# jtdaugherty/flux

Hardware: AMD Instinct MI355X
Metric: Msamples/sec on demo2.yml (fixed spp) (higher is better)
Workload: dtype f64

## Files before the change

flux_amd/_lib.py:

```python
import ctypes as C
import os

_HERE = os.path.dirname(os.path.abspath(__file__))
LIB_PATH = os.environ.get("FLUX_HIP_LIB") or os.path.join(_HERE, "libflux_hip.so")

FLUX_OK = 0
E_INVALID, E_DEVICE, E_NOMEM, E_IO = -1, -2, -3, -4
SHAPE_SPHERE, SHAPE_PLANE, SHAPE_DISK, SHAPE_BOX = 0, 1, 2, 3
MAT_MATTE, MAT_EMISSIVE, MAT_REFLECTIVE, MAT_GLOSSY = 0, 1, 2, 3
MAT_DIELECTRIC = 4
KERNEL_DEFAULT, KERNEL_STATIC, KERNEL_REFILL, KERNEL_SPLIT = 0, 1, 2, 3
MATH_FAST, MATH_STRICT = 0, 1
SAMPLER_REGULAR, SAMPLER_JITTERED, SAMPLER_MULTI_JITTERED, SAMPLER_CORRELATED_MULTI_JITTERED = 0, 1, 2, 3
TABLE_PIXEL, TABLE_DISC, TABLE_HEMI = 0, 1, 2
TRAVERSE_BVH, TRAVERSE_BRUTE, TRAVERSE_BVH_BINARY = 0, 1, 2
NUM_STATS = 16
BVH_INFO_WORDS = 16
PLAN_WORDS = 8
PLAN_NONE, PLAN_STATIC, PLAN_REFILL, PLAN_SPLIT, PLAN_BVH_BINARY, PLAN_BVH4 = -1, 0, 1, 2, 3, 4
ROUTE_NONE, ROUTE_TO_STRICT, ROUTE_KEPT_FAST = 0, 1, 2
PLAN_FLAG_TYP, PLAN_FLAG_MAX32, PLAN_FLAG_HITQ, PLAN_FLAG_TPUT_TABLE = 0x1, 0x2, 0x4, 0x8
PLAN_FLAG_DEPTH_CUT, PLAN_FLAG_UNIFORM_A, PLAN_FLAG_LDS_SCENE, PLAN_FLAG_TRIS = 0x10, 0x20, 0x40, 0x80
PLAN_FLAG_AXIS_SHIFT, PLAN_FLAG_AXIS_MASK = 8, 0x300
PLAN_FLAG_HQ_BITS_SHIFT, PLAN_FLAG_HQ_BITS_MASK = 10, 0xfc00
PLAN_FLAG_COPY_SHIFT, PLAN_FLAG_COPY_MASK = 16, 0x30000
CREATE_TIMING_WORDS = 8
CREATE_TIMING_NAMES = ("total", "host", "runtime", "alloc", "upload", "tables", "free", "other")
SHARD_AUTO, SHARD_SETS, SHARD_ROWS = 0, 1, 2
SHARD_LOOPBACK = 0x100
MULTI_INFO_WORDS = 8
MULTI_TIMING_WORDS = 8
ABI_VERSION = 3
AOV_CHANNELS = 8
AOV_ALBEDO_OFFSET, AOV_NORMAL_OFFSET, AOV_DEPTH, AOV_COVERAGE = 0, 3, 6, 7
AOV_ALBEDO, AOV_NORMAL = slice(AOV_ALBEDO_OFFSET, AOV_ALBEDO_OFFSET + 3), slice(AOV_NORMAL_OFFSET, AOV_NORMAL_OFFSET + 3)
MOMENT_CHANNELS = 8
MOMENT_RGB_OFFSET, MOMENT_VAR, MOMENT_MEAN_OFFSET, MOMENT_S2 = 0, 3, 4, 7
# ... 164 lines not shown
```

flux_amd/build.py:

```python
import os
import shutil
import subprocess
import sys

ROOT = os.path.dirname(os.path.dirname(os.path.abspath(__file__)))
CSRC = os.path.join(ROOT, "flux_amd", "csrc")
HIP_SOURCES = ["abi.hip", "multi.hip", "tables.hip", "render.hip", "denoise.hip", "adaptive.hip", "bvh.cpp", "scene_build.cpp", "launch_plan.cpp"]
HIP_HEADERS = ["flux_ctx.h", "scene_build.h", "joining_thread.h", "flux_device.h", "flux_plan.h", "flux_rng.h", "flux_tables.h", "flux_bvh.h", "flux_math.h",
               "flux_math_coeffs.h", "flux_env_verdict.h", "flux_plane_axis.h", "flux_moments.h", "render_body.inc", "aov_body.inc", "moments_body.inc", "adaptive_body.inc", "aov_chain_body.inc"]
HIP_LIB = os.path.join(ROOT, "flux_amd", "libflux_hip.so")

HIP_FLAGS = ["--offload-arch=gfx950", "-O3", "-std=c++17", "-fPIC", "-shared", "-ffp-contract=off",
             "-fno-fast-math", "-Wall", "-Wno-unused-function",
             "-mllvm", "-disable-machine-licm"]


def _newer(target, deps):
    if not os.path.exists(target):
        return True
    t = os.path.getmtime(target)
    return any(os.path.getmtime(d) > t for d in deps)


def _hipcc():
    for cand in (os.environ.get("HIPCC"), shutil.which("hipcc"), "/opt/rocm/bin/hipcc"):
        if cand and os.path.exists(cand):
            return cand
    raise RuntimeError("hipcc not found (set HIPCC)")


KERNEL_FILES = ["render.hip", "render_body.inc", "aov_body.inc", "moments_body.inc", "adaptive_body.inc", "aov_chain_body.inc", "tables.hip", "denoise.hip", "adaptive.hip", "flux_device.h", "flux_plan.h", "flux_bvh.h", "flux_math.h",
                "flux_math_coeffs.h", "flux_rng.h", "flux_tables.h", "flux_env_verdict.h", "flux_plane_axis.h", "flux_moments.h"]


def build_id(extra_flags=()):
    import hashlib

    def digest(names):
        h = hashlib.sha256()
        h.update(" ".join(HIP_FLAGS + list(extra_flags)).encode())
        for n in names:
            path = os.path.join(ROOT, "include", n) if n == "flux_abi.h" else os.path.join(CSRC, n)
            h.update(n.encode() + b"\0")
            with open(path, "rb") as f:
                h.update(f.read())
        return h.hexdigest()[:16]
    return f"lib:{digest(sorted(set(HIP_SOURCES + HIP_HEADERS + ['flux_abi.h'])))} kernels:{digest(KERNEL_FILES)}"


def _id_flag(extra_flags=()):
    return "-DFLUX_BUILD_ID=\"" + build_id(extra_flags) + "\""


def build_variant(out_path, extra_flags, verbose=False):
    srcs = [os.path.join(CSRC, s) for s in HIP_SOURCES]
# ... 48 lines not shown
```

flux_amd/csrc/abi.hip:

```cpp
#include <hip/hip_runtime.h>

#include <chrono>
#include <cmath>
#include <cstdarg>
#include <cstdio>
#include <cstring>
#include <memory>
#include <new>
#include <algorithm>
#include <cstdlib>
#include <string>
#include <vector>

#include "../../include/flux_abi.h"
#include "flux_device.h"
#include "flux_tables.h"
#include "flux_math_coeffs.h"

#include "flux_ctx.h"

namespace flux {

thread_local std::string g_last_error;

// ... 184 lines not shown
    const char *tables_env = std::getenv("FLUX_SAMPLE_TABLES");
    const int gx_stride = (tables_env && std::atoi(tables_env) == 0) ? 0 : h.rp.gx_stride;
    if (gx_stride) {
        alloc(c->d_glossx, own * c->N * (size_t)gx_stride);
        alloc_copy(c->d_gxoff, h.gx_off);
    }
    int tput_bits = 0;
    bool tput_finite = false;
    {
        RenderParams job = h.rp;
        job.nsamp = c->N;
        job.max_depth = (int32_t)c->D;
        const char *tput_env = std::getenv("FLUX_THROUGHPUT_TABLE");
        if (tput_table_bytes(job, &tput_bits)) {
            std::vector<double> tput;
            build_tput_table(h, tput_bits, (int)c->D, tput);
            tput_finite = tput_products_finite(h, tput_bits, (int)c->D, tput);
            if (!(tput_env && std::atoi(tput_env) == 0)) alloc_copy(c->d_tput, tput);
        }
    }
    std::vector<unsigned char> lobe_entries;
    const size_t lobe_bytes = lobe_frame_table(h, lobe_entries);
    if (lobe_bytes) alloc(c->d_lobe, lobe_bytes);
    alloc(c->d_setrows, own * sizeof(DevSetRows));
    alloc(c->d_rowperm, perm_bytes);
    alloc(c->d_invperm, perm_bytes);
    alloc(c->d_stats, FLUX_NUM_STATS * sizeof(unsigned long long));
    if (!h.tris.empty()) {
        alloc_copy(c->d_tris, h.tris);
        alloc_copy(c->d_nodes, h.nodes);
        alloc_copy(c->d_nodesq, h.nodesq);
        if (!h.arena.empty()) alloc_copy(c->d_arena, h.arena);
    }
    if (e == hipSuccess) e = hipMemset(c->d_stats, 0, FLUX_NUM_STATS * sizeof(unsigned long long));
    laps.lap(FLUX_CREATE_MS_UPLOAD);
    if (e == hipSuccess) e = c->ev0.create();
    if (e == hipSuccess) e = c->ev1.create();
    laps.lap(FLUX_CREATE_MS_OTHER);
    double tab_ms[3] = {0, 0, 0};
    if (e == hipSuccess)
        e = generate_tables(seed, c->S, c->sets, c->D, c->n, c->H, c->d_pix, c->d_disc, c->d_hemi, c->d_rowperm, c->d_invperm, nullptr, tab_ms);
    if (e == hipSuccess) {
        e = generate_gloss_table(c->d_pix, (size_t)c->sets.count * c->N, c->d_gloss, nullptr);
        if (e == hipSuccess && gx_stride)
            e = generate_glossx_table(c->d_gloss, (size_t)c->sets.count * c->N, h.gx_inv_e1.data(), h.rp.n_gloss_exp, gx_stride / 16,
                                      c->d_glossx, nullptr);
        if (e == hipSuccess && c->d_lobe)
            e = generate_lobe_frame_table(reinterpret_cast<const DevHitRec *>(c->d_fscene + h.fs.rec), (int)lobe_entries.size(), c->d_lobe, nullptr);
        if (e == hipSuccess) e = hipStreamSynchronize(nullptr);
    }
    laps.lap(FLUX_CREATE_MS_TABLES);
    laps.ms[FLUX_CREATE_MS_TABLES] -= tab_ms[0] + tab_ms[2];
    laps.ms[FLUX_CREATE_MS_ALLOC] += tab_ms[0];
    laps.ms[FLUX_CREATE_MS_FREE] += tab_ms[2];
    if (e == hipSuccess) {
        std::vector<DevSetRows> rows(own, DevSetRows{});
        for (size_t m = 0; m < own; m++) {
            rows[m].pix = c->d_pix + m * c->N;
            rows[m].disc = c->d_disc + m * c->N;
            rows[m].hemi = c->d_hemi + m * c->D * c->N * kHemiDoubles;
            rows[m].gloss = c->d_gloss + m * c->N * 4;
            rows[m].glossx = gx_stride ? c->d_glossx + m * c->N * (size_t)(gx_stride / 16) : nullptr;
        }
        copy(c->d_setrows, rows);
    }
    if (e != hipSuccess)
        return fail(e == hipErrorOutOfMemory ? FLUX_E_NOMEM : FLUX_E_DEVICE, "flux_ctx_create: %s", hipGetErrorString(e));

    RenderParams &rp = c->rp;
    rp = h.rp;
    rp.pixel_denom = 1.0 / (double)((uint64_t)c->n * c->n);
    rp.max_depth = (int32_t)c->D;
    rp.nsamp = c->N;
    rp.shapes = c->d_shapes;
    rp.mats = c->d_mats;
    rp.pix = c->d_pix;
    rp.disc = c->d_disc;
    rp.hemi = c->d_hemi;
    rp.gloss = c->d_gloss;
    rp.glossx = c->d_glossx;
    rp.gx_off = c->d_gxoff;
    rp.gx_stride = gx_stride;
    rp.tput = c->d_tput;
    rp.tput_bits = c->d_tput ? tput_bits : 0;
// ... 587 lines not shown
    return FLUX_OK;
}

int flux_ctx_copy_table(flux_ctx *ctx, int which, double *out, uint64_t out_doubles) {
    if (!ctx || !out) return fail(FLUX_E_INVALID, "null argument");
    DeviceGuard guard(ctx->device);
    const size_t SN = (size_t)ctx->sets.count * ctx->N;
    if (which == FLUX_TABLE_PIXEL || which == FLUX_TABLE_DISC) {
        if (out_doubles < SN * 2) return fail(FLUX_E_INVALID, "output too small: need %zu doubles", SN * 2);
        HIP_TRY(hipMemcpy(out, which == FLUX_TABLE_PIXEL ? ctx->d_pix : ctx->d_disc, SN * 2 * sizeof(double),
                          hipMemcpyDeviceToHost));
        return FLUX_OK;
    }
    if (which == FLUX_TABLE_HEMI) {
        const size_t total = SN * ctx->D * 3;
        if (out_doubles < total) return fail(FLUX_E_INVALID, "output too small: need %zu doubles", total);
        flux::DevBuf<double> tmp;
        HIP_TRY(tmp.alloc(total));
        hipError_t e = flux::hemi_to_aos((size_t)ctx->sets.count * ctx->D, ctx->N, ctx->d_hemi, tmp, nullptr);
        if (e == hipSuccess) e = hipMemcpy(out, tmp, total * sizeof(double), hipMemcpyDeviceToHost);
        if (e != hipSuccess) return fail(FLUX_E_DEVICE, "hemi copy: %s", hipGetErrorString(e));
        return FLUX_OK;
    }
    return fail(FLUX_E_INVALID, "unknown table %d", which);
}

int flux_ctx_copy_row_perm(flux_ctx *ctx, uint64_t row, int32_t *out, uint64_t out_len) {
    if (!ctx || !out) return fail(FLUX_E_INVALID, "null argument");
    if (row >= ctx->H) return fail(FLUX_E_INVALID, "row %llu outside image height %u", (unsigned long long)row, ctx->H);
    if (out_len < ctx->S) return fail(FLUX_E_INVALID, "output too small: need %u entries", ctx->S);
    DeviceGuard guard(ctx->device);
    HIP_TRY(hipMemcpy(out, ctx->d_rowperm + (size_t)row * ctx->S, (size_t)ctx->S * sizeof(int32_t),
                      hipMemcpyDeviceToHost));
    return FLUX_OK;
}

int flux_ctx_camera_basis(flux_ctx *ctx, double uvw[9]) {
    if (!ctx || !uvw) return fail(FLUX_E_INVALID, "null argument");
    for (int i = 0; i < 3; i++) {
        uvw[i] = ctx->U[i];
        uvw[3 + i] = ctx->V[i];
        uvw[6 + i] = ctx->Wv[i];
    }
    return FLUX_OK;
}

// ... 61 lines not shown
```

flux_amd/csrc/flux_ctx.h:

```cpp
#pragma once
#include <hip/hip_runtime.h>

#include <chrono>
#include <new>
#include <optional>
#include <string>
#include <system_error>
#include <utility>

#include "../../include/flux_abi.h"
#include "flux_device.h"
#include "flux_tables.h"
#include "scene_build.h"

namespace flux {

extern thread_local std::string g_last_error;
int fail(int code, const char *fmt, ...) __attribute__((format(printf, 2, 3)));

template <class F> int no_throw(F &&f) {
    try {
        return f();
    } catch (const std::bad_alloc &) {
        return fail(FLUX_E_NOMEM, "host allocation failed");
// ... 88 lines not shown
        if (e_ != hipSuccess)                                                                     \
            return flux::fail(e_ == hipErrorOutOfMemory ? FLUX_E_NOMEM : FLUX_E_DEVICE, "%s: %s", \
                              #expr, hipGetErrorString(e_));                                      \
    } while (0)

struct flux_ctx {
    std::optional<flux::DeviceGuard> dying;
    ~flux_ctx() { dying.emplace(device); }
    int device = 0;
    flux::RenderParams rp{};
    uint64_t seed = 0;
    uint32_t n = 0, N = 0, D = 0, S = 0, W = 0, H = 0;
    flux::SetRange sets{0, 1, 0};
    flux::DevBuf<flux::DevShape> d_shapes;
    flux::DevBuf<flux::DevMaterial> d_mats;
    flux::DevBuf<unsigned char> d_fscene;
    flux::DevBuf<double2> d_pix, d_disc;
    flux::DevBuf<double> d_hemi;
    flux::DevBuf<double> d_gloss;
    flux::DevBuf<double2> d_glossx;
    flux::DevBuf<int32_t> d_gxoff;
    flux::DevBuf<double> d_tput;
    flux::DevBuf<double> d_lobe;
    flux::DevBuf<flux::DevSetRows> d_setrows;
    flux::DevBuf<int32_t> d_rowperm, d_invperm;
    flux::DevBuf<unsigned long long> d_stats;
    bool stats_on = false;
    flux::DevBuf<flux::DevTri> d_tris;
    flux::DevBuf<flux::DevNode> d_nodes;
    flux::DevBuf<flux::DevNode4A> d_arena;
    flux::DevBuf<flux::DevNodeQ> d_nodesq;
    flux::BvhInfo bvh{};
    int traversal = FLUX_TRAVERSE_BVH;
    int variant = FLUX_KERNEL_DEFAULT;
    int math = FLUX_MATH_FAST;
    flux::Scratch<double> d_out, d_aov, d_moments, d_aov_chain;
    flux::DevBuf<double> d_adapt_sums, d_adapt_out;
    flux::DevBuf<uint32_t> d_adapt_passes, d_adapt_list, d_adapt_counts, d_adapt_map;
    flux::DevBuf<unsigned char> d_adapt_hot;
    flux::Capacity d_adapt_pixels, d_adapt_out_pixels;
    flux::Event ev0, ev1;
    bool timed = false;
    uint64_t device_bytes = 0;
    double U[3], V[3], Wv[3];
    double create_ms[FLUX_CREATE_TIMING_WORDS] = {};
};
// ... 1 lines not shown
```

flux_amd/csrc/flux_device.h:

```cpp
#pragma once
#include <hip/hip_runtime.h>
#include <stdint.h>

#include "flux_bvh.h"
#include "flux_env_verdict.h"
#include "flux_plane_axis.h"


#ifndef FLUX_UNI_SPHERES
#define FLUX_UNI_SPHERES 2
#endif
#ifndef FLUX_BVH_WIDE_MAX_STACK
#define FLUX_BVH_WIDE_MAX_STACK 48
#endif
#ifndef FLUX_MAX_WAVES_PER_PIXEL
#define FLUX_MAX_WAVES_PER_PIXEL 4
#endif
#ifndef FLUX_MIN_SAMPLES_PER_WAVE
#define FLUX_MIN_SAMPLES_PER_WAVE 4096
#endif

namespace flux {

constexpr int kHemiDoubles = 4;
// ... 68 lines not shown
    double inv;
};
static_assert(sizeof(DevScanBox) == 64, "DevScanBox layout");
struct DevHitRec {
    double cx, cy, cz;
    double inv_rad;
    double fr, fg, fb;
    double inv_e1;
    int32_t shape_kind, mat_kind;
    int32_t orig_id;
    int32_t unit_normal;
    double ax, az;
};
static_assert(sizeof(DevHitRec) == 96, "DevHitRec layout");

struct SetRange {
    uint32_t first, stride, count;
};

struct DevSetRows {
    const double2 *pix, *disc;
    const double *hemi, *gloss;
    const double2 *glossx;
    const void *pad[3];
};
static_assert(sizeof(DevSetRows) == 64, "DevSetRows layout");

struct RenderParams {
    double ex, ey, ez;
    double Ux, Uy, Uz, Vx, Vy, Vz, Wx, Wy, Wz;
    double aps;
    double half_w, half_h;
    double factor;
    double focal, lens_radius;
    double bgr, bgg, bgb;
    double pixel_denom;
    int32_t img_w, img_h;
    int32_t n_shapes, max_depth;
    uint32_t nsamp;
    uint32_t num_sets;
    const DevShape *shapes;
    const DevMaterial *mats;
    const double2 *pix;
    const double2 *disc;
    const double *hemi;
    const double *gloss;
    const int32_t *rowperm;
// ... 72 lines not shown
```

flux_amd/csrc/flux_tables.h:

```cpp
#pragma once
#include <hip/hip_runtime.h>
#include <stdint.h>
#include "flux_device.h"
#include "flux_plan.h"

namespace flux {

hipError_t generate_tables(uint64_t seed, uint32_t S, SetRange sets, uint32_t D, uint32_t n, uint32_t H,
                           double2 *pix, double2 *disc, double *hemi, int32_t *rowperm, int32_t *invperm,
                           hipStream_t stream, double *phase_ms = nullptr);
hipError_t generate_sampler_grid(int kind, uint64_t seed, uint32_t n, double *d_xy, double *d_hemi,
                                 hipStream_t stream);
hipError_t generate_gloss_table(const double2 *pix, size_t count, double *gloss, hipStream_t stream);
hipError_t generate_glossx_table(const double *gloss, size_t count, const double *inv_e1, int n, int pad, double2 *out, hipStream_t stream);
hipError_t generate_lobe_frame_table(const DevHitRec *frec, int n_rec, double *out, hipStream_t stream);
hipError_t hemi_to_aos(size_t SD, size_t N, const double *in, double *out, hipStream_t stream);

hipError_t launch_pass(Pass pass, const RenderParams &p, int variant, int math, hipStream_t stream);

hipError_t launch_adaptive(const RenderParams &p, const AdaptiveWork &a, int math, hipStream_t stream);
hipError_t launch_aov_chain(const RenderParams &p, int max_chain, int math, hipStream_t stream);

struct AdaptiveRule {
    double tau2, lum_floor;
    uint32_t nsamp, dilate;
};
hipError_t launch_adaptive_select(const AdaptiveRule &rule, uint32_t rows, uint32_t width, const double *sums, const uint32_t *passes,
                                  unsigned char *hot, uint32_t *list, uint32_t *count, hipStream_t stream);
hipError_t launch_adaptive_finish(uint32_t nsamp, uint64_t pixels, const double *sums, const uint32_t *passes, double *out_moments,
                                  uint32_t *out_passes, hipStream_t stream);
hipError_t launch_adaptive_count(uint32_t max_passes, uint64_t pixels, const uint32_t *passes, uint32_t *reached, hipStream_t stream);

hipError_t launch_shade_rays(const RenderParams &p, int math, const double *d_rays, int n, int depth, uint32_t set,
// ... 9 lines not shown
```

flux_amd/csrc/render_body.inc:

```

#undef FLUX_STAGE
#if FLUX_FAST
#define FLUX_STAGE() __builtin_amdgcn_sched_barrier(0)
#else
#define FLUX_STAGE() ((void)0)
#endif

struct Ray {
    double ox, oy, oz, dx, dy, dz;
};

typedef const __attribute__((address_space(4))) RenderParams *ParamsInKernarg;
static_assert(sizeof(DevMaterial) % 16 == 0, "the bounce-weight records behind the materials are read as double2");
__device__ __forceinline__ const RenderParams &relaunder_params(uint32_t tick) {
    ParamsInKernarg p = (ParamsInKernarg)__builtin_amdgcn_kernarg_segment_ptr();
    asm("" : "+s"(p) : "s"(tick));
    return *(const RenderParams *)p;
}

struct SplitDepths {
    int max_depth, cut_depth;
};
constexpr bool split_depth_pair(bool TYP) { return TYP; }
template <bool PAIR>
// ... 1922 lines not shown
        const uint32_t C = (uint32_t)hq_cap, H = (uint32_t)hq_th;
        const uint32_t bmask = (1u << hq_bits) - 1u;
        const DevHitRec *const recs = reinterpret_cast<const DevHitRec *>(frec_lds);
        uint32_t *const pool = reinterpret_cast<uint32_t *>(q);
        uint32_t next = s_lo;
        uint32_t nhit = 0;
        constexpr int kDeadDepth = 0x7fffffff;
        for (;;) {
            const RenderParams &P = relaunder_params(next + nhit);
            uint32_t set_p = set;
            unsigned long long cand_p = cand_mask, in_p = in_mask;
            asm("" : "+s"(set_p) : "s"(next));
            asm("" : "+s"(cand_p), "+s"(in_p) : "s"(next));
            Path p;
            path_begin(p);
            p.depth = kDeadDepth;
            p.sq = make_double2(0.5, 0.5);
            uint32_t i = 0;
            uint32_t ml = 0;
            const bool run_a = next < s_hi && nhit < H && hitq_admits_phase_a(C, nhit);
            if (run_a) {
                FLUX_TRIP(P, 12);
                FLUX_CENSUS(P, 0);
                const uint32_t ia = next + lane;
                const bool valid = ia < s_hi;
                const unsigned long long valid_m = ballot64(ia < s_hi);
                next = (s_hi - next) > 64u ? next + 64u : s_hi;
                bool cont = false;
                const double2 *pix = set_rows_of(P, set_p).pix;
                const double2 *disc = set_rows_of(P, set_p).disc;
                const char *pxc_b = reinterpret_cast<const char *>(P.pxc);
                const PixelConsts PX = PixelConsts{*reinterpret_cast<const double *>(pxc_b + ((uint32_t)col << 3)),
                                                   *reinterpret_cast<const double *>(pxc_b + ((uint32_t)(P.img_w + row) << 3)), P.fwx, P.fwy, P.fwz};
                {
                    const uint32_t ic = ia < s_hi ? ia : s_hi - 1u;
                    p.sq = gather_global_d2(pix, ic << 4);
                    p.r = primary_ray_px(P, PX, p.sq, gather_global_d2(disc, ic << 4));
                    if (STATS && valid) {
                        st.c[0]++;
                        st.c[1]++;
                    }
                }
                int hit = -1;
                double t = 0.0;
                scan_shapes_primary<TYP, AXIS>(P, p.r, cand_p, in_p, in_t0, valid, valid_m, hit, t);
                p.depth = 1;
                if (valid) {
                    double Lr, Lg, Lb;
                    FLUX_CENSUS(P, 2);
                    cont = shade_primary_hits<STATS, TYP, split_uniform_a(TYP, HQ), split_lobe_frames(MAX32, TYP, HQ)>(P, p, set_p, ia, hit, t, Lr, Lg, Lb, st, frec_lds, uni_a);
                    if (cont && p.depth > P.max_depth) {
                        cont = false;
                        Lr = Lg = Lb = 0.0;
                        if (STATS) st.c[7]++;
                    }
                    if (!cont) {
                        fold_path(p, nullptr, 0, Lr, Lg, Lb);
                        sr += Lr;
                        sg += Lg;
                        sb += Lb;
// ... 142 lines not shown
                if (p.depth == kDeadDepth && rank < take) {
                    const uint32_t slot = qcount - 1u - rank;
                    p.r.ox = q[0 * 64 + slot];
                    p.r.oy = q[1 * 64 + slot];
                    p.r.oz = q[2 * 64 + slot];
                    p.r.dx = q[3 * 64 + slot];
                    p.r.dy = q[4 * 64 + slot];
                    p.r.dz = q[5 * 64 + slot];
                    p.tr = q[6 * 64 + slot];
                    p.tg = q[7 * 64 + slot];
                    p.tb = q[8 * 64 + slot];
                    i = (uint32_t)qi[slot];
                    p.self = qi[64 + slot];
                    p.depth = 2;
                    p.nb = 1;
                }
                qcount -= take;
            };
            pop();
            lap_stamp(lap, 0);
            if (next < s_hi && any64(p.depth == kDeadDepth)) {
                FLUX_TRIP(P, 12);
                FLUX_CENSUS(P, 0);
                const uint32_t ia = next + lane;
                const bool valid = ia < s_hi;
                const unsigned long long valid_m = ballot64(ia < s_hi);
                next = (s_hi - next) > 64u ? next + 64u : s_hi;
                bool cont = false;
                Path pa;
                path_begin(pa);
                pa.sq = make_double2(0.5, 0.5);
                pa.r = Ray{0, 0, 0, 0, 0, 1};
                const double2 *pix = set_rows_of(P, set_p).pix;
                const double2 *disc = set_rows_of(P, set_p).disc;
                const char *pxc_b = reinterpret_cast<const char *>(P.pxc);
                const PixelConsts PX = PixelConsts{*reinterpret_cast<const double *>(pxc_b + ((uint32_t)col << 3)),
                                                   *reinterpret_cast<const double *>(pxc_b + ((uint32_t)(P.img_w + row) << 3)), P.fwx, P.fwy, P.fwz};
                {
                    const uint32_t ic = ia < s_hi ? ia : s_hi - 1u;
                    pa.sq = gather_global_d2(pix, ic << 4);
                    pa.r = primary_ray_px(P, PX, pa.sq, gather_global_d2(disc, ic << 4));
                    if (STATS && valid) {
                        st.c[0]++;
                        st.c[1]++;
                    }
                }
                int hit = -1;
                double t = 0.0;
                scan_shapes_primary<TYP, AXIS>(P, pa.r, cand_p, in_p, in_t0, valid, valid_m, hit, t);
                if (valid) {
                    double Lr, Lg, Lb;
                    FLUX_CENSUS(P, 2);
                    cont = shade_primary_hits<STATS, TYP, split_uniform_a(TYP, HQ), split_lobe_frames(MAX32, TYP, HQ)>(P, pa, set_p, ia, hit, t, Lr, Lg, Lb, st, frec_lds, uni_a);
                    if (cont && pa.depth > P.max_depth) {
                        cont = false;
                        Lr = Lg = Lb = 0.0;
                        if (STATS) st.c[7]++;
                    }
                    if (!cont) {
                        fold_path(pa, nullptr, 0, Lr, Lg, Lb);
                        sr += Lr;
                        sg += Lg;
                        sb += Lb;
                    }
// ... 823 lines not shown
```

flux_amd/csrc/tables.hip:

```cpp
#include <chrono>

#include "flux_device.h"
#include "flux_rng.h"
#include "flux_tables.h"

namespace flux {

__device__ __forceinline__ uint32_t global_set(SetRange sets, uint32_t slot) { return sets.first + slot * sets.stride; }

__global__ void cmj_perm_kernel(uint64_t seed, uint64_t kind, SetRange sets, uint32_t n, uint16_t *perms) {
    uint32_t t = blockIdx.x * blockDim.x + threadIdx.x;
    if (t >= sets.count * 2u) return;
    uint32_t s = t >> 1, which = t & 1u;
    shuffle_iota(stream_key(seed, kind, global_set(sets, s), 0, 1 + which), perms + (size_t)t * n, n);
}

__global__ void mj_perm_kernel(uint64_t seed, SetRange sets, uint32_t D, uint32_t n, uint16_t *perms) {
    size_t t = (size_t)blockIdx.x * blockDim.x + threadIdx.x;
    size_t total = (size_t)sets.count * D * 2u * n;
    if (t >= total) return;
    uint32_t sub = (uint32_t)(t % (2u * n));
    size_t sd = t / (2u * n);
    uint32_t d = (uint32_t)(sd % D), s = (uint32_t)(sd / D);
    shuffle_iota(stream_key(seed, kKindHemi, global_set(sets, s), d, 1 + sub), perms + t * n, n);
}

__global__ void row_perm_kernel(uint64_t seed, uint32_t H, uint32_t S, int32_t *rowperm) {
// ... 180 lines not shown
        (void)hipFree(cmj_perms);
        return e;
    }
    uint16_t *pix_perms = cmj_perms, *disc_perms = cmj_perms + cmj_elems;
    const unsigned bs = 256;
    lap(0);
    cmj_perm_kernel<<<blocks_for((size_t)So * 2, 64), 64, 0, stream>>>(seed, kKindPixel, sets, n, pix_perms);
    cmj_perm_kernel<<<blocks_for((size_t)So * 2, 64), 64, 0, stream>>>(seed, kKindDisc, sets, n, disc_perms);
    mj_perm_kernel<<<blocks_for((size_t)So * D * 2 * n, bs), bs, 0, stream>>>(seed, sets, D, n, mj_perms);
    row_perm_kernel<<<blocks_for(H, 64), 64, 0, stream>>>(seed, H, S, rowperm);
    inv_perm_kernel<<<blocks_for((size_t)H * S, bs), bs, 0, stream>>>(H, S, rowperm, invperm);
    cmj_fill_kernel<<<blocks_for((size_t)So * N, bs), bs, 0, stream>>>(seed, kKindPixel, sets, n, pix_perms, pix);
    cmj_fill_kernel<<<blocks_for((size_t)So * N, bs), bs, 0, stream>>>(seed, kKindDisc, sets, n, disc_perms, disc);
    hemi_fill_kernel<<<blocks_for((size_t)So * D * N, bs), bs, 0, stream>>>(seed, sets, D, n, mj_perms, hemi);
    e = hipGetLastError();
    hipError_t e2 = hipStreamSynchronize(stream);
    lap(1);
    (void)hipFree(cmj_perms);
    (void)hipFree(mj_perms);
    lap(2);
    return e != hipSuccess ? e : e2;
}

hipError_t hemi_to_aos(size_t SD, size_t N, const double *in, double *out, hipStream_t stream) {
    hemi_to_aos_kernel<<<blocks_for(SD * N, 256), 256, 0, stream>>>(SD, N, in, out);
    return hipGetLastError();
}

}
```

flux_amd/render.py:

```python
import ctypes as C

import numpy as np

from . import _lib
from .scene import JobConfiguration, SceneData, SceneDesc, WorkUnit, WorkUnitResult

STAT_NAMES = ("samples", "segments", "matte_bounces", "glossy_bounces", "specular_bounces",
              "emissive_hits", "misses", "depth_exhausted", "bvh_nodes", "tris_tested",
              "dielectric_reflections", "dielectric_transmissions")


class Renderer:
    def __init__(self, scene_data: SceneData, config: JobConfiguration, seed: int = 1, device: int = 0,
                 set_share=None):
        self.scene_data = scene_data
        self.config = config
        self.seed = int(seed)
        self.device = int(device)
        self.width = scene_data.output_settings.image_width
        self.height = scene_data.output_settings.image_height
        self._desc = SceneDesc(scene_data)
        cfg = _lib.FluxJobCfg(config.sample_root, config.max_trace_depth, config.rows_per_work_unit)
        h = C.c_void_p()
        self.set_share = (0, 1) if set_share is None else (int(set_share[0]), int(set_share[1]))
# ... 220 lines not shown
        _lib.check(_lib.lib.flux_ctx_stats(self._handle(), buf, 0))
        return [int(x) for x in buf]

    def set_traversal(self, mode: int):
        _lib.check(_lib.lib.flux_ctx_set_traversal(self._handle(), mode))

    def bvh_info(self) -> dict:
        buf = (C.c_uint64 * _lib.BVH_INFO_WORDS)()
        _lib.check(_lib.lib.flux_ctx_bvh_info(self._handle(), buf, _lib.BVH_INFO_WORDS))
        names = ("nodes", "triangles", "max_depth", "max_leaf", "node_bytes", "tri_bytes", "build_us", "wide_nodes",
                 "leaf_records", "fused_leaves", "wide_stack", "wide_node_bytes", "leaf_record_bytes", "wide_in_use")
        return dict(zip(names, [int(x) for x in buf]))

    def launch_plan(self, num_rows=None, num_sets: int = 0, flags: bool = False) -> dict:
        buf = (C.c_int64 * _lib.PLAN_WORDS)()
        _lib.check(_lib.lib.flux_ctx_launch_plan(self._handle(), self.height if num_rows is None else num_rows, num_sets, buf))
        names = ("kernel", "block", "blocks", "lds", "waves_per_pixel", "math", "route") + (("flags",) if flags else ())
        return dict(zip(names, [int(x) for x in buf]))

    def table(self, which: int) -> np.ndarray:
        S = len(range(self.set_share[0], self.width, self.set_share[1]))
        N = self.config.sample_root ** 2
        D = self.config.max_trace_depth
        shape = (S, N, 2) if which in (_lib.TABLE_PIXEL, _lib.TABLE_DISC) else (S, D, N, 3)
        out = np.empty(shape, dtype=np.float64)
        _lib.check(_lib.lib.flux_ctx_copy_table(self._handle(), which, out.ctypes.data_as(C.POINTER(C.c_double)),
                                                out.size))
        return out

    def row_perm(self, row: int) -> np.ndarray:
        out = np.empty(self.width, dtype=np.int32)
        _lib.check(_lib.lib.flux_ctx_copy_row_perm(self._handle(), row, out.ctypes.data_as(C.POINTER(C.c_int32)),
                                                   out.size))
        return out

    def camera_basis(self) -> np.ndarray:
        out = np.empty(9, dtype=np.float64)
        _lib.check(_lib.lib.flux_ctx_camera_basis(self._handle(), out.ctypes.data_as(C.POINTER(C.c_double))))
        return out.reshape(3, 3)

    def device_bytes(self) -> int:
        return int(_lib.lib.flux_ctx_device_bytes(self._handle()))

    def create_timing(self) -> dict:
        return _create_timing(self._handle())


# ... 208 lines not shown
```

include/flux_abi.h:

```cpp
#ifndef FLUX_ABI_H
#define FLUX_ABI_H

#include <stddef.h>
#include <stdint.h>

#ifdef __cplusplus
extern "C" {
#endif

#define FLUX_ABI_VERSION 3

#define FLUX_OK 0
#define FLUX_E_INVALID (-1)
#define FLUX_E_DEVICE (-2)
#define FLUX_E_NOMEM (-3)
#define FLUX_E_IO (-4)

#define FLUX_SHAPE_SPHERE 0
#define FLUX_SHAPE_PLANE 1
#define FLUX_SHAPE_DISK 2
#define FLUX_SHAPE_BOX 3

#define FLUX_MAT_MATTE 0
#define FLUX_MAT_EMISSIVE 1
// ... 171 lines not shown
#define FLUX_PLAN_FLAG_LDS_SCENE 0x40u
#define FLUX_PLAN_FLAG_TRIS 0x80u
#define FLUX_PLAN_FLAG_AXIS_SHIFT 8
#define FLUX_PLAN_FLAG_AXIS_MASK 0x300u
#define FLUX_PLAN_FLAG_HQ_BITS_SHIFT 10
#define FLUX_PLAN_FLAG_HQ_BITS_MASK 0xfc00u
#define FLUX_PLAN_FLAG_COPY_SHIFT 16
#define FLUX_PLAN_FLAG_COPY_MASK 0x30000u
#define FLUX_ROUTE_NONE 0
#define FLUX_ROUTE_TO_STRICT 1
#define FLUX_ROUTE_KEPT_FAST 2
#define FLUX_PLAN_NONE (-1)
#define FLUX_PLAN_STATIC 0
#define FLUX_PLAN_REFILL 1
#define FLUX_PLAN_SPLIT 2
#define FLUX_PLAN_BVH_BINARY 3
#define FLUX_PLAN_BVH4 4
#define FLUX_PLAN_WORDS 8
int flux_ctx_launch_plan(flux_ctx *ctx, uint64_t num_rows, uint64_t num_sets, int64_t out[FLUX_PLAN_WORDS]);

#define FLUX_TABLE_PIXEL 0
#define FLUX_TABLE_DISC 1
#define FLUX_TABLE_HEMI 2
int flux_ctx_copy_table(flux_ctx *ctx, int which, double *out, uint64_t out_doubles);
int flux_ctx_copy_row_perm(flux_ctx *ctx, uint64_t row, int32_t *out, uint64_t out_len);
int flux_ctx_camera_basis(flux_ctx *ctx, double uvw[9]);
uint64_t flux_ctx_device_bytes(flux_ctx *ctx);

#define FLUX_CREATE_MS_TOTAL 0
#define FLUX_CREATE_MS_HOST 1
#define FLUX_CREATE_MS_RUNTIME 2
#define FLUX_CREATE_MS_ALLOC 3
#define FLUX_CREATE_MS_UPLOAD 4
#define FLUX_CREATE_MS_TABLES 5
#define FLUX_CREATE_MS_FREE 6
#define FLUX_CREATE_MS_OTHER 7
#define FLUX_CREATE_TIMING_WORDS 8
int flux_ctx_create_timing(flux_ctx *ctx, double out_ms[FLUX_CREATE_TIMING_WORDS]);

#define FLUX_SAMPLER_REGULAR 0
#define FLUX_SAMPLER_JITTERED 1
#define FLUX_SAMPLER_MULTI_JITTERED 2
#define FLUX_SAMPLER_CORRELATED_MULTI_JITTERED 3
int flux_sampler_grid(int device, int kind, uint64_t sample_root, uint64_t seed, double *out_xy, double *out_hemi);

int flux_debug_shade(flux_ctx *ctx, uint64_t n, const double *rays, uint64_t depth, uint64_t set_index,
// ... 47 lines not shown
```

Baseline: 58620.

## Reorder per-set samples by first-bounce hemisphere direction for wave coherence

Adds a per-set sample order computed at context creation. Samples are sorted by a Morton key of the first hemisphere sample's direction, then dealt in groups of 64 across the four wave slices. Pixel and disc tables are pre-permuted so the render kernel reads them contiguously, and it indirects through the order to get the sample index used for later-bounce hemisphere lookups. The goal is for each wave's lanes to follow similar secondary-ray directions, which should reduce divergence in BVH traversal and shading. In exchange it costs an extra gather per refill, more device memory, and a sort at setup.

After: 62890, median of 6. 1.07x the previous value.

```diff
diff --git a/flux_amd/_lib.py b/flux_amd/_lib.py
--- a/flux_amd/_lib.py
+++ b/flux_amd/_lib.py
@@ -12,7 +12,7 @@
 KERNEL_DEFAULT, KERNEL_STATIC, KERNEL_REFILL, KERNEL_SPLIT = 0, 1, 2, 3
 MATH_FAST, MATH_STRICT = 0, 1
 SAMPLER_REGULAR, SAMPLER_JITTERED, SAMPLER_MULTI_JITTERED, SAMPLER_CORRELATED_MULTI_JITTERED = 0, 1, 2, 3
-TABLE_PIXEL, TABLE_DISC, TABLE_HEMI = 0, 1, 2
+TABLE_PIXEL, TABLE_DISC, TABLE_HEMI, TABLE_ORDER = 0, 1, 2, 3
 TRAVERSE_BVH, TRAVERSE_BRUTE, TRAVERSE_BVH_BINARY = 0, 1, 2
 NUM_STATS = 16
 BVH_INFO_WORDS = 16
diff --git a/flux_amd/build.py b/flux_amd/build.py
--- a/flux_amd/build.py
+++ b/flux_amd/build.py
@@ -7,7 +7,7 @@
 CSRC = os.path.join(ROOT, "flux_amd", "csrc")
 HIP_SOURCES = ["abi.hip", "multi.hip", "tables.hip", "render.hip", "denoise.hip", "adaptive.hip", "bvh.cpp", "scene_build.cpp", "launch_plan.cpp"]
 HIP_HEADERS = ["flux_ctx.h", "scene_build.h", "joining_thread.h", "flux_device.h", "flux_plan.h", "flux_rng.h", "flux_tables.h", "flux_bvh.h", "flux_math.h",
-               "flux_math_coeffs.h", "flux_env_verdict.h", "flux_plane_axis.h", "flux_moments.h", "render_body.inc", "aov_body.inc", "moments_body.inc", "adaptive_body.inc", "aov_chain_body.inc"]
+               "flux_math_coeffs.h", "flux_env_verdict.h", "flux_plane_axis.h", "flux_sample_order.h", "flux_moments.h", "render_body.inc", "aov_body.inc", "moments_body.inc", "adaptive_body.inc", "aov_chain_body.inc"]
 HIP_LIB = os.path.join(ROOT, "flux_amd", "libflux_hip.so")
 
 HIP_FLAGS = ["--offload-arch=gfx950", "-O3", "-std=c++17", "-fPIC", "-shared", "-ffp-contract=off",
@@ -30,7 +30,7 @@
 
 
 KERNEL_FILES = ["render.hip", "render_body.inc", "aov_body.inc", "moments_body.inc", "adaptive_body.inc", "aov_chain_body.inc", "tables.hip", "denoise.hip", "adaptive.hip", "flux_device.h", "flux_plan.h", "flux_bvh.h", "flux_math.h",
-                "flux_math_coeffs.h", "flux_rng.h", "flux_tables.h", "flux_env_verdict.h", "flux_plane_axis.h", "flux_moments.h"]
+                "flux_math_coeffs.h", "flux_rng.h", "flux_tables.h", "flux_env_verdict.h", "flux_plane_axis.h", "flux_sample_order.h", "flux_moments.h"]
 
 
 def build_id(extra_flags=()):
diff --git a/flux_amd/csrc/abi.hip b/flux_amd/csrc/abi.hip
--- a/flux_amd/csrc/abi.hip
+++ b/flux_amd/csrc/abi.hip
@@ -230,6 +230,9 @@
     std::vector<unsigned char> lobe_entries;
     const size_t lobe_bytes = lobe_frame_table(h, lobe_entries);
     if (lobe_bytes) alloc(c->d_lobe, lobe_bytes);
+    alloc(c->d_order, own * c->N * sizeof(uint32_t));
+    alloc(c->d_pix_o, pix_bytes);
+    alloc(c->d_disc_o, pix_bytes);
     alloc(c->d_setrows, own * sizeof(DevSetRows));
     alloc(c->d_rowperm, perm_bytes);
     alloc(c->d_invperm, perm_bytes);
@@ -256,6 +259,11 @@
         if (e == hipSuccess && c->d_lobe)
             e = generate_lobe_frame_table(reinterpret_cast<const DevHitRec *>(c->d_fscene + h.fs.rec), (int)lobe_entries.size(), c->d_lobe, nullptr);
         if (e == hipSuccess) e = hipStreamSynchronize(nullptr);
+        const char *order_env = std::getenv("FLUX_SAMPLE_ORDER");
+        if (e == hipSuccess)
+            e = generate_sample_order(c->sets.count, c->D, c->n, c->d_hemi, c->d_order, order_env && std::atoi(order_env) == 0, nullptr, tab_ms);
+        if (e == hipSuccess)
+            e = generate_order_copies((size_t)c->sets.count * c->N, c->N, c->d_order, c->d_pix, c->d_disc, c->d_pix_o, c->d_disc_o, nullptr);
     }
     laps.lap(FLUX_CREATE_MS_TABLES);
     laps.ms[FLUX_CREATE_MS_TABLES] -= tab_ms[0] + tab_ms[2];
@@ -268,6 +276,9 @@
             rows[m].disc = c->d_disc + m * c->N;
             rows[m].hemi = c->d_hemi + m * c->D * c->N * kHemiDoubles;
             rows[m].gloss = c->d_gloss + m * c->N * 4;
+            rows[m].order = c->d_order + m * c->N;
+            rows[m].pix_o = c->d_pix_o + m * c->N;
+            rows[m].disc_o = c->d_disc_o + m * c->N;
             rows[m].glossx = gx_stride ? c->d_glossx + m * c->N * (size_t)(gx_stride / 16) : nullptr;
         }
         copy(c->d_setrows, rows);
@@ -901,6 +912,15 @@
         if (e != hipSuccess) return fail(FLUX_E_DEVICE, "hemi copy: %s", hipGetErrorString(e));
         return FLUX_OK;
     }
+    if (which == FLUX_TABLE_ORDER) {
+        if (out_doubles < SN) return fail(FLUX_E_INVALID, "output too small: need %zu doubles", SN);
+        return flux::no_throw([&]() -> int {
+            std::vector<uint32_t> tmp(SN);
+            HIP_TRY(hipMemcpy(tmp.data(), ctx->d_order, SN * sizeof(uint32_t), hipMemcpyDeviceToHost));
+            for (size_t k = 0; k < SN; k++) out[k] = (double)tmp[k];
+            return FLUX_OK;
+        });
+    }
     return fail(FLUX_E_INVALID, "unknown table %d", which);
 }
 
diff --git a/flux_amd/csrc/flux_ctx.h b/flux_amd/csrc/flux_ctx.h
--- a/flux_amd/csrc/flux_ctx.h
+++ b/flux_amd/csrc/flux_ctx.h
@@ -134,6 +134,8 @@
     flux::DevBuf<int32_t> d_gxoff;
     flux::DevBuf<double> d_tput;
     flux::DevBuf<double> d_lobe;
+    flux::DevBuf<double2> d_pix_o, d_disc_o;
+    flux::DevBuf<uint32_t> d_order;
     flux::DevBuf<flux::DevSetRows> d_setrows;
     flux::DevBuf<int32_t> d_rowperm, d_invperm;
     flux::DevBuf<unsigned long long> d_stats;
diff --git a/flux_amd/csrc/flux_device.h b/flux_amd/csrc/flux_device.h
--- a/flux_amd/csrc/flux_device.h
+++ b/flux_amd/csrc/flux_device.h
@@ -114,7 +114,8 @@
     const double2 *pix, *disc;
     const double *hemi, *gloss;
     const double2 *glossx;
-    const void *pad[3];
+    const uint32_t *order;
+    const double2 *pix_o, *disc_o;
 };
 static_assert(sizeof(DevSetRows) == 64, "DevSetRows layout");
 
diff --git a/flux_amd/csrc/flux_sample_order.h b/flux_amd/csrc/flux_sample_order.h
--- /dev/null
+++ b/flux_amd/csrc/flux_sample_order.h
@@ -0,0 +1,73 @@
+#pragma once
+#include <stdint.h>
+
+#include <vector>
+
+#if defined(__HIPCC__) || defined(__CUDACC__)
+#define FLUX_SO_HD __host__ __device__ inline
+#else
+#define FLUX_SO_HD inline
+#endif
+
+namespace flux {
+
+constexpr uint32_t kOrderCellBits = 7;
+constexpr uint32_t kOrderKeyBits = 2 * kOrderCellBits;
+constexpr uint32_t kOrderGroup = 64;
+constexpr uint32_t kOrderQuarters = 4;
+
+FLUX_SO_HD uint32_t order_cell(double v) {
+    const double s = (v + 1.0) * 64.0;
+    if (!(s > 0.0)) return 0u;
+    if (s >= 127.0) return 127u;
+    return (uint32_t)s;
+}
+
+FLUX_SO_HD uint32_t order_spread(uint32_t v) {
+    v &= 0x7fu;
+    v = (v | (v << 4)) & 0x0f0fu;
+    v = (v | (v << 2)) & 0x3333u;
+    v = (v | (v << 1)) & 0x5555u;
+    return v;
+}
+
+FLUX_SO_HD uint32_t order_key(double x, double y) { return order_spread(order_cell(x)) | (order_spread(order_cell(y)) << 1); }
+
+FLUX_SO_HD uint32_t order_slice_lo(uint32_t N, uint32_t sub, uint32_t K) { return (uint32_t)((uint64_t)N * sub / K); }
+
+struct OrderDeal {
+    uint32_t N;
+    uint32_t fill[kOrderQuarters];
+    FLUX_SO_HD explicit OrderDeal(uint32_t n) : N(n), fill{0u, 0u, 0u, 0u} {}
+    FLUX_SO_HD uint32_t groups() const { return (N + kOrderGroup - 1u) / kOrderGroup; }
+    template <class F>
+    FLUX_SO_HD void group(uint32_t g, F &&f) {
+        const uint32_t first = g * kOrderGroup;
+        uint32_t left = N - first < kOrderGroup ? N - first : kOrderGroup, e0 = 0u;
+        uint32_t q = g % kOrderQuarters;
+        while (left) {
+            const uint32_t lo = order_slice_lo(N, q, kOrderQuarters), hi = order_slice_lo(N, q + 1u, kOrderQuarters);
+            const uint32_t room = hi - lo - fill[q];
+            const uint32_t take = room < left ? room : left;
+            if (take) f(e0, take, lo + fill[q]);
+            fill[q] += take;
+            e0 += take;
+            left -= take;
+            q = (q + 1u) % kOrderQuarters;
+        }
+    }
+};
+
+template <class Keys, class Index, class StableSort>
+inline void order_row_host(const Keys &keys, uint32_t N, Index *row, StableSort &&stable_sort_by_key) {
+    std::vector<Index> sorted(N);
+    for (uint32_t i = 0; i < N; i++) sorted[i] = (Index)i;
+    stable_sort_by_key(sorted.data(), sorted.data() + N, keys);
+    OrderDeal deal(N);
+    for (uint32_t g = 0; g < deal.groups(); g++)
+        deal.group(g, [&](uint32_t e0, uint32_t count, uint32_t pos) {
+            for (uint32_t k = 0; k < count; k++) row[pos + k] = sorted[g * kOrderGroup + e0 + k];
+        });
+}
+
+}
diff --git a/flux_amd/csrc/flux_tables.h b/flux_amd/csrc/flux_tables.h
--- a/flux_amd/csrc/flux_tables.h
+++ b/flux_amd/csrc/flux_tables.h
@@ -9,6 +9,10 @@
 hipError_t generate_tables(uint64_t seed, uint32_t S, SetRange sets, uint32_t D, uint32_t n, uint32_t H,
                            double2 *pix, double2 *disc, double *hemi, int32_t *rowperm, int32_t *invperm,
                            hipStream_t stream, double *phase_ms = nullptr);
+hipError_t generate_sample_order(uint32_t sets, uint32_t D, uint32_t n, const double *hemi, uint32_t *order, bool identity,
+                                 hipStream_t stream, double *phase_ms = nullptr);
+hipError_t generate_order_copies(size_t count, uint32_t N, const uint32_t *order, const double2 *pix, const double2 *disc, double2 *pix_o,
+                                 double2 *disc_o, hipStream_t stream);
 hipError_t generate_sampler_grid(int kind, uint64_t seed, uint32_t n, double *d_xy, double *d_hemi,
                                  hipStream_t stream);
 hipError_t generate_gloss_table(const double2 *pix, size_t count, double *gloss, hipStream_t stream);
diff --git a/flux_amd/csrc/render_body.inc b/flux_amd/csrc/render_body.inc
--- a/flux_amd/csrc/render_body.inc
+++ b/flux_amd/csrc/render_body.inc
@@ -1968,20 +1968,21 @@
             if (run_a) {
                 FLUX_TRIP(P, 12);
                 FLUX_CENSUS(P, 0);
-                const uint32_t ia = next + lane;
-                const bool valid = ia < s_hi;
-                const unsigned long long valid_m = ballot64(ia < s_hi);
+                const uint32_t slot_a = next + lane;
+                const bool valid = slot_a < s_hi;
+                const unsigned long long valid_m = ballot64(slot_a < s_hi);
+                const uint32_t kc_a = slot_a < s_hi ? slot_a : s_hi - 1u;
+                const uint32_t ia = gather_global<uint32_t>(set_rows_of(P, set_p).order, kc_a << 2);
                 next = (s_hi - next) > 64u ? next + 64u : s_hi;
                 bool cont = false;
-                const double2 *pix = set_rows_of(P, set_p).pix;
-                const double2 *disc = set_rows_of(P, set_p).disc;
+                const double2 *pix = set_rows_of(P, set_p).pix_o;
+                const double2 *disc = set_rows_of(P, set_p).disc_o;
                 const char *pxc_b = reinterpret_cast<const char *>(P.pxc);
                 const PixelConsts PX = PixelConsts{*reinterpret_cast<const double *>(pxc_b + ((uint32_t)col << 3)),
                                                    *reinterpret_cast<const double *>(pxc_b + ((uint32_t)(P.img_w + row) << 3)), P.fwx, P.fwy, P.fwz};
                 {
-                    const uint32_t ic = ia < s_hi ? ia : s_hi - 1u;
-                    p.sq = gather_global_d2(pix, ic << 4);
-                    p.r = primary_ray_px(P, PX, p.sq, gather_global_d2(disc, ic << 4));
+                    p.sq = gather_global_d2(pix, kc_a << 4);
+                    p.r = primary_ray_px(P, PX, p.sq, gather_global_d2(disc, kc_a << 4));
                     if (STATS && valid) {
                         st.c[0]++;
                         st.c[1]++;
@@ -2170,24 +2171,25 @@
             if (next < s_hi && any64(p.depth == kDeadDepth)) {
                 FLUX_TRIP(P, 12);
                 FLUX_CENSUS(P, 0);
-                const uint32_t ia = next + lane;
-                const bool valid = ia < s_hi;
-                const unsigned long long valid_m = ballot64(ia < s_hi);
+                const uint32_t slot_a = next + lane;
+                const bool valid = slot_a < s_hi;
+                const unsigned long long valid_m = ballot64(slot_a < s_hi);
+                const uint32_t kc_a = slot_a < s_hi ? slot_a : s_hi - 1u;
+                const uint32_t ia = gather_global<uint32_t>(set_rows_of(P, set_p).order, kc_a << 2);
                 next = (s_hi - next) > 64u ? next + 64u : s_hi;
                 bool cont = false;
                 Path pa;
                 path_begin(pa);
                 pa.sq = make_double2(0.5, 0.5);
                 pa.r = Ray{0, 0, 0, 0, 0, 1};
-                const double2 *pix = set_rows_of(P, set_p).pix;
-                const double2 *disc = set_rows_of(P, set_p).disc;
+                const double2 *pix = set_rows_of(P, set_p).pix_o;
+                const double2 *disc = set_rows_of(P, set_p).disc_o;
                 const char *pxc_b = reinterpret_cast<const char *>(P.pxc);
                 const PixelConsts PX = PixelConsts{*reinterpret_cast<const double *>(pxc_b + ((uint32_t)col << 3)),
                                                    *reinterpret_cast<const double *>(pxc_b + ((uint32_t)(P.img_w + row) << 3)), P.fwx, P.fwy, P.fwz};
                 {
-                    const uint32_t ic = ia < s_hi ? ia : s_hi - 1u;
-                    pa.sq = gather_global_d2(pix, ic << 4);
-                    pa.r = primary_ray_px(P, PX, pa.sq, gather_global_d2(disc, ic << 4));
+                    pa.sq = gather_global_d2(pix, kc_a << 4);
+                    pa.r = primary_ray_px(P, PX, pa.sq, gather_global_d2(disc, kc_a << 4));
                     if (STATS && valid) {
                         st.c[0]++;
                         st.c[1]++;
diff --git a/flux_amd/csrc/tables.hip b/flux_amd/csrc/tables.hip
--- a/flux_amd/csrc/tables.hip
+++ b/flux_amd/csrc/tables.hip
@@ -1,8 +1,14 @@
+#include <algorithm>
 #include <chrono>
-
+#include <vector>
+
+#include "flux_ctx.h"
 #include "flux_device.h"
 #include "flux_rng.h"
+#include "flux_sample_order.h"
 #include "flux_tables.h"
+
+#include <rocprim/device/device_segmented_radix_sort.hpp>
 
 namespace flux {
 
@@ -229,6 +235,107 @@
     return e != hipSuccess ? e : e2;
 }
 
+static_assert(kOrderQuarters == FLUX_MAX_WAVES_PER_PIXEL && kOrderGroup == 64, "the deal's quarters are the split kernel's slices, its groups a wave's batch");
+__global__ void order_key_kernel(size_t count, uint32_t D, uint32_t N, const double *__restrict__ hemi, uint16_t *__restrict__ keys,
+                                 uint32_t *__restrict__ index) {
+    const size_t t = (size_t)blockIdx.x * blockDim.x + threadIdx.x;
+    if (t >= count) return;
+    const size_t s = t / N;
+    const uint32_t i = (uint32_t)(t - s * N);
+    const double *h = hemi + ((s * D) * N + i) * kHemiDoubles;
+    keys[t] = (uint16_t)order_key(h[0], h[1]);
+    index[t] = i;
+}
+
+__global__ __launch_bounds__(kOrderGroup) void order_deal_kernel(uint32_t N, const uint32_t *__restrict__ sorted, uint32_t *__restrict__ order) {
+    const uint32_t lane = threadIdx.x;
+    const uint32_t *src = sorted + (size_t)blockIdx.x * N;
+    uint32_t *dst = order + (size_t)blockIdx.x * N;
+    OrderDeal deal(N);
+    for (uint32_t g = 0; g < deal.groups(); g++)
+        deal.group(g, [&](uint32_t e0, uint32_t count, uint32_t pos) {
+            if (lane >= e0 && lane - e0 < count) dst[pos + (lane - e0)] = src[g * kOrderGroup + lane];
+        });
+}
+
+__global__ void order_identity_kernel(size_t count, uint32_t N, uint32_t *__restrict__ order) {
+    const size_t t = (size_t)blockIdx.x * blockDim.x + threadIdx.x;
+    if (t < count) order[t] = (uint32_t)(t % N);
+}
+
+__global__ void order_copies_kernel(size_t count, uint32_t N, const uint32_t *__restrict__ order, const double2 *__restrict__ pix,
+                                    const double2 *__restrict__ disc, double2 *__restrict__ pix_o, double2 *__restrict__ disc_o) {
+    const size_t t = (size_t)blockIdx.x * blockDim.x + threadIdx.x;
+    if (t >= count) return;
+    const size_t src = t / N * N + order[t];
+    pix_o[t] = pix[src];
+    disc_o[t] = disc[src];
+}
+hipError_t generate_order_copies(size_t count, uint32_t N, const uint32_t *order, const double2 *pix, const double2 *disc, double2 *pix_o,
+                                 double2 *disc_o, hipStream_t stream) {
+    if (count == 0) return hipSuccess;
+    order_copies_kernel<<<blocks_for(count, 256), 256, 0, stream>>>(count, N, order, pix, disc, pix_o, disc_o);
+    const hipError_t e = hipGetLastError(), e2 = hipStreamSynchronize(stream);
+    return e != hipSuccess ? e : e2;
+}
+
+hipError_t generate_sample_order(uint32_t sets, uint32_t D, uint32_t n, const double *hemi, uint32_t *order, bool identity,
+                                 hipStream_t stream, double *phase_ms) {
+    const uint32_t N = n * n;
+    if (sets == 0) return hipSuccess;
+    auto t_last = std::chrono::steady_clock::now();
+    auto lap = [&](int k) {
+        const auto now = std::chrono::steady_clock::now();
+        if (phase_ms) phase_ms[k] += std::chrono::duration<double, std::milli>(now - t_last).count();
+        t_last = now;
+    };
+    if (identity) {
+        order_identity_kernel<<<blocks_for((size_t)sets * N, 256), 256, 0, stream>>>((size_t)sets * N, N, order);
+        const hipError_t e = hipGetLastError(), e2 = hipStreamSynchronize(stream);
+        lap(1);
+        return e != hipSuccess ? e : e2;
+    }
+    const uint32_t chunk = std::min<uint32_t>(sets, std::max<uint32_t>(1u, (1u << 24) / N));
+    const size_t elems = (size_t)chunk * N;
+    std::vector<uint32_t> offs(chunk + 1u);
+    for (uint32_t m = 0; m <= chunk; m++) offs[m] = m * N;
+    DevBuf<uint16_t> keys_in, keys_out;
+    DevBuf<uint32_t> idx_in, idx_out, d_offs;
+    DevBuf<unsigned char> temp;
+    size_t temp_bytes = 0;
+    hipError_t e = keys_in.alloc(elems);
+    if (e == hipSuccess) e = keys_out.alloc(elems);
+    if (e == hipSuccess) e = idx_in.alloc(elems);
+    if (e == hipSuccess) e = idx_out.alloc(elems);
+    if (e == hipSuccess) e = d_offs.alloc(chunk + 1u);
+    if (e == hipSuccess)
+        e = rocprim::segmented_radix_sort_pairs(nullptr, temp_bytes, (uint16_t *)keys_in, (uint16_t *)keys_out, (uint32_t *)idx_in,
+                                                (uint32_t *)idx_out, (unsigned int)elems, chunk, (uint32_t *)d_offs, (uint32_t *)d_offs + 1, 0u,
+                                                kOrderKeyBits, stream);
+    if (e == hipSuccess) e = temp.alloc(temp_bytes ? temp_bytes : 1);
+    if (e == hipSuccess) e = hipMemcpyAsync(d_offs, offs.data(), offs.size() * sizeof(uint32_t), hipMemcpyHostToDevice, stream);
+    lap(0);
+    for (uint32_t m0 = 0; m0 < sets && e == hipSuccess; m0 += chunk) {
+        const uint32_t m = std::min(chunk, sets - m0);
+        const size_t count = (size_t)m * N;
+        order_key_kernel<<<blocks_for(count, 256), 256, 0, stream>>>(count, D, N, hemi + (size_t)m0 * D * N * kHemiDoubles, keys_in, idx_in);
+        e = hipGetLastError();
+        if (e == hipSuccess)
+            e = rocprim::segmented_radix_sort_pairs((void *)(unsigned char *)temp, temp_bytes, (uint16_t *)keys_in, (uint16_t *)keys_out,
+                                                    (uint32_t *)idx_in, (uint32_t *)idx_out, (unsigned int)count, m, (uint32_t *)d_offs,
+                                                    (uint32_t *)d_offs + 1, 0u, kOrderKeyBits, stream);
+        if (e == hipSuccess) {
+            order_deal_kernel<<<m, kOrderGroup, 0, stream>>>(N, idx_out, order + (size_t)m0 * N);
+            e = hipGetLastError();
+        }
+    }
+    const hipError_t e2 = hipStreamSynchronize(stream);
+    lap(1);
+    keys_in.reset(), keys_out.reset(), idx_in.reset(), idx_out.reset(), d_offs.reset(), temp.reset();
+    lap(2);
+    return e != hipSuccess ? e : e2;
+}
+
 hipError_t hemi_to_aos(size_t SD, size_t N, const double *in, double *out, hipStream_t stream) {
     hemi_to_aos_kernel<<<blocks_for(SD * N, 256), 256, 0, stream>>>(SD, N, in, out);
     return hipGetLastError();
diff --git a/flux_amd/render.py b/flux_amd/render.py
--- a/flux_amd/render.py
+++ b/flux_amd/render.py
@@ -266,7 +266,7 @@
         S = len(range(self.set_share[0], self.width, self.set_share[1]))
         N = self.config.sample_root ** 2
         D = self.config.max_trace_depth
-        shape = (S, N, 2) if which in (_lib.TABLE_PIXEL, _lib.TABLE_DISC) else (S, D, N, 3)
+        shape = (S, N, 2) if which in (_lib.TABLE_PIXEL, _lib.TABLE_DISC) else (S, N) if which == _lib.TABLE_ORDER else (S, D, N, 3)
         out = np.empty(shape, dtype=np.float64)
         _lib.check(_lib.lib.flux_ctx_copy_table(self._handle(), which, out.ctypes.data_as(C.POINTER(C.c_double)),
                                                 out.size))
diff --git a/include/flux_abi.h b/include/flux_abi.h
--- a/include/flux_abi.h
+++ b/include/flux_abi.h
@@ -217,6 +217,7 @@
 #define FLUX_TABLE_PIXEL 0
 #define FLUX_TABLE_DISC 1
 #define FLUX_TABLE_HEMI 2
+#define FLUX_TABLE_ORDER 3
 int flux_ctx_copy_table(flux_ctx *ctx, int which, double *out, uint64_t out_doubles);
 int flux_ctx_copy_row_perm(flux_ctx *ctx, uint64_t row, int32_t *out, uint64_t out_len);
 int flux_ctx_camera_basis(flux_ctx *ctx, double uvw[9]);
```
